# davidbau/rewriting

Measured on NVIDIA H100. Metric: StyleGAN2-256 images/sec, higher is better.
Workload: dtype bf16x3 (3-term split bf16 operands, fp32 accumulate; fp32 in/out)

## Files before the change

rewriting_b200/csrc/conv_tc.cu:

```cuda
#include <cstdlib>
#include <cstring>

#include "rw_common.cuh"
#include "rw_kernels.h"

namespace rw {

namespace {

constexpr int BM = 128;
constexpr int BN = 128;
constexpr int BK = 32;
constexpr int MMA_K = 16;
constexpr int kStages = 7;
constexpr int kNumThreads = 384;
constexpr int kTmaWarp = 8;
constexpr uint32_t kProducerRegs = 40;
constexpr uint32_t kConsumerRegs = 232;
constexpr int kCluster = 2;
constexpr int kChunkKB = 16;

struct ConvSmem {
  static constexpr int kABytes = BM * BK * 2;
  static constexpr int kBBytes = BN * BK * 2;
  static constexpr int kStageBytes = 2 * kABytes + 2 * kBBytes;
  static constexpr int kTotal = kStages * kStageBytes + 512  + 256 ;
};
static_assert(ConvSmem::kTotal <= 232448, "conv_tc: shared memory over the per-block limit");

struct Barriers {
  uint64_t full[kStages];
  uint64_t empty[kStages];
};

__device__ __forceinline__ void decode_tile(int tile, int nphase, int nsched, int& ph, int& mn) {
  mn = tile / nphase;
  ph = tile - mn * nphase;
  if (nphase > 1) ph = (ph + ((nsched % nphase) == 0 ? tile / nsched : mn)) % nphase;
}

template <int EPI, bool PROF>
__global__ void __launch_bounds__(kNumThreads, 1)
conv_tc_kernel(const __grid_constant__ CUtensorMap map_a_hi,
               const __grid_constant__ CUtensorMap map_a_lo,
               const __grid_constant__ CUtensorMap map_w_hi,
               const __grid_constant__ CUtensorMap map_w_lo, const ConvTcParams p) {
  extern __shared__ uint8_t smem_raw[];
  uint8_t* smem = reinterpret_cast<uint8_t*>((reinterpret_cast<uintptr_t>(smem_raw) + 511) &
                                             ~static_cast<uintptr_t>(511));
  using S = ConvSmem;
  Barriers* bars = reinterpret_cast<Barriers*>(smem + kStages * S::kStageBytes);

  const int warp = __shfl_sync(0xffffffffu, static_cast<int>(threadIdx.x >> 5), 0);
  const int lane = threadIdx.x & 31;
  const int rank = static_cast<int>(cluster_ctarank());
  const int nsched = static_cast<int>(num_clusters_x());
  const int first_unit = static_cast<int>(cluster_id_x());

  const int m_tiles = (p.rows + BM - 1) / BM;
  const int n_tiles = p.Cout / BN;
  const int mn_units = (m_tiles + kCluster - 1) / kCluster * n_tiles;
  const int num_units = mn_units * p.nphase;
  const int kb_per_tap = p.Cin / BK;

  if (warp == kTmaWarp && lane == 0) {
    tma_prefetch_desc(&map_a_hi);
    tma_prefetch_desc(&map_a_lo);
    tma_prefetch_desc(&map_w_hi);
    tma_prefetch_desc(&map_w_lo);
    for (int s = 0; s < kStages; ++s) {
      mbar_init(&bars->full[s], 1);
      mbar_init(&bars->empty[s], 2 * kCluster);
    }
    fence_mbar_init();
  }
  cluster_sync();

  if (warp < kTmaWarp) {
    setmaxnreg_inc<kConsumerRegs>();
    const int wg = threadIdx.x >> 7;
    const int c = lane & 3;
    const int img = p.Hp * p.Wp;
    auto release = [&](int s) {
      if ((threadIdx.x & 127) == 0) {
#pragma unroll
        for (int r = 0; r < kCluster; ++r) mbar_arrive_cluster(mapa_shared(&bars->empty[s], r));
      }
    };
    auto clk = [] { return static_cast<uint32_t>(clock()); };
    uint32_t prof[6] = {0, 0, 0, 0, 0, 0};
    uint32_t tp0 = 0, tp1 = 0;
    if constexpr (PROF) prof[5] = 0u - clk();
    int stage = 0;
    uint32_t phase = 0;
    for (int unit = first_unit; unit < num_units; unit += nsched) {
      int ph, mn;
      decode_tile(unit, p.nphase, nsched, ph, mn);
      const int num_kb = p.ph_ntaps[ph] * kb_per_tap;
      const int n_tile = mn % n_tiles;
      const int n0 = n_tile * BN;
      const int m0 = ((mn / n_tiles) * kCluster + rank) * BM;

      float acc[64], d[64];
#pragma unroll
      for (int j = 0; j < 64; ++j) acc[j] = 0.f;
      for (int kb0 = 0; kb0 < num_kb; kb0 += kChunkKB) {
        const int kb_end = (kb0 + kChunkKB < num_kb) ? kb0 + kChunkKB : num_kb;
        int held = -1;
        for (int kb = kb0; kb < kb_end; ++kb) {
          if constexpr (PROF) tp0 = clk();
          mbar_wait(&bars->full[stage], phase);
          if constexpr (PROF) { tp1 = clk(); prof[0] += tp1 - tp0; }
          const uint32_t sa = smem_u32(smem + stage * S::kStageBytes);
          const uint64_t da_hi = make_smem_desc(sa + wg * (S::kABytes / 2), 16, 512, 2);
          const uint64_t da_lo = make_smem_desc(sa + S::kABytes + wg * (S::kABytes / 2), 16, 512, 2);
          const uint64_t db_hi = make_smem_desc(sa + 2 * S::kABytes, 16, 512, 2);
          const uint64_t db_lo = make_smem_desc(sa + 2 * S::kABytes + S::kBBytes, 16, 512, 2);
          wgmma_fence();
#pragma unroll
          for (int kk = 0; kk < BK / MMA_K; ++kk) {
            const uint64_t adv = static_cast<uint64_t>((kk * MMA_K * 2) >> 4);
            wgmma_m64n128<0, 0>(d, da_lo + adv, db_hi + adv, ((kb - kb0) | kk) != 0);
            wgmma_m64n128<0, 0>(d, da_hi + adv, db_lo + adv, 1u);
            wgmma_m64n128<0, 0>(d, da_hi + adv, db_hi + adv, 1u);
          }
          wgmma_commit();
          wgmma_wait<1>();
          if (held >= 0) release(held);
          held = stage;
          if (++stage == kStages) { stage = 0; phase ^= 1u; }
          if constexpr (PROF) prof[1] += clk() - tp1;
        }
        if constexpr (PROF) tp0 = clk();
        wgmma_wait<0>();
        release(held);
#pragma unroll
        for (int j = 0; j < 64; ++j) acc[j] += d[j];
        if constexpr (PROF) prof[2] += clk() - tp0;
      }
      if constexpr (PROF) tp0 = clk();

      uint32_t tid;
      asm volatile("mov.u32 %0, %%tid.x;\n" : "=r"(tid));
      const int row0 = m0 + ((tid >> 7) << 6) + (((tid >> 5) & 3) << 4) + ((tid & 31) >> 2);
#pragma unroll
      for (int i = 0; i < 2; ++i) {
        const int prow = row0 + 8 * i;
        const int b = prow / img;
        const int rem = prow - b * img;
        const int yy = rem / p.Wp;
        const int xx = rem - yy * p.Wp;
        const int Hv = p.ph_Hv[ph], Wv = p.ph_Wv[ph];
        const bool in_rows = prow < p.rows;
        const bool valid = in_rows && (yy < Hv) && (xx < Wv);
        const float* scl = (p.scale_bo && in_rows) ? p.scale_bo + static_cast<size_t>(b) * p.Cout : nullptr;
        float* outp = (p.out != nullptr && p.out_mode == 0 && valid)
                          ? p.out + p.ph_out_ofs[ph] + static_cast<size_t>(b) * p.out_sb +
                                static_cast<size_t>(yy) * p.out_sy + static_cast<size_t>(xx) * p.out_sx
                          : nullptr;
        if (EPI == 1 || !valid) {
          if (scl && (EPI == 1 || p.out_mode == 1)) {
#pragma unroll
            for (int j = 0; j < 16; ++j) {
              const float2 sv = __ldg(reinterpret_cast<const float2*>(scl + n0 + 8 * j + 2 * c));
              acc[4 * j + 2 * i] *= sv.x;
              acc[4 * j + 2 * i + 1] *= sv.y;
            }
          }
          if (EPI == 1 && outp) {
#pragma unroll
            for (int j = 0; j < 16; ++j)
#pragma unroll
              for (int e = 0; e < 2; ++e)
                outp[static_cast<size_t>(n0 + 8 * j + 2 * c + e) * p.out_sc] = acc[4 * j + 2 * i + e];
          }
        } else {
          float nz = 0.f;
          if (p.noise != nullptr)
            nz = __ldg(p.noise_w) * __ldg(p.noise + static_cast<size_t>(b) * p.noise_bstride +
                                          static_cast<size_t>(yy) * Wv + xx);
          const float act_gain = p.act_gain != 0.f ? p.act_gain : 1.4142135623730951f;
          if (scl) {
            const float* sc = scl + n0 + 2 * c;
#pragma unroll
            for (int j = 0; j < 16; ++j)
#pragma unroll
              for (int e = 0; e < 2; ++e) acc[4 * j + 2 * i + e] *= __ldg(sc + 8 * j + e);
          }
#pragma unroll
          for (int j = 0; j < 16; ++j)
#pragma unroll
            for (int e = 0; e < 2; ++e) acc[4 * j + 2 * i + e] += nz;
          if (p.bias) {
            const float* bi = p.bias + n0 + 2 * c;
#pragma unroll
            for (int j = 0; j < 16; ++j)
#pragma unroll
              for (int e = 0; e < 2; ++e) acc[4 * j + 2 * i + e] += __ldg(bi + 8 * j + e);
          }
          if (p.act) {
#pragma unroll
            for (int j = 0; j < 32; ++j) {
              float& t = acc[4 * (j >> 1) + 2 * i + (j & 1)];
              t = (t > 0.f ? t : 0.2f * t) * act_gain;
            }
          }
          if (outp) {
#pragma unroll
            for (int j = 0; j < 16; ++j)
#pragma unroll
              for (int e = 0; e < 2; ++e)
                outp[static_cast<size_t>(n0 + 8 * j + 2 * c + e) * p.out_sc] = acc[4 * j + 2 * i + e];
          }
        }
        if (EPI == 0 && p.rgb_w != nullptr) {
          const float* rw0 = p.rgb_w + (static_cast<size_t>(valid ? b : 0) * 3) * p.Cout + n0 + 2 * c;
          const float* rw1 = rw0 + p.Cout;
          const float* rw2 = rw1 + p.Cout;
#pragma unroll
          for (int half = 0; half < 2; ++half) {
            float r0 = 0.f, r1 = 0.f, r2 = 0.f;
            if (valid) {
#pragma unroll
              for (int j = 8 * half; j < 8 * half + 8; ++j)
#pragma unroll
                for (int e = 0; e < 2; ++e) {
                  const float t = acc[4 * j + 2 * i + e];
                  r0 = fmaf(__ldg(rw0 + 8 * j + e), t, r0);
                  r1 = fmaf(__ldg(rw1 + 8 * j + e), t, r1);
                  r2 = fmaf(__ldg(rw2 + 8 * j + e), t, r2);
                }
            }
#pragma unroll
            for (int s = 1; s < 4; s <<= 1) {
              r0 += __shfl_xor_sync(0xffffffffu, r0, s);
              r1 += __shfl_xor_sync(0xffffffffu, r1, s);
              r2 += __shfl_xor_sync(0xffffffffu, r2, s);
            }
            if (valid && c == 0) {
              const size_t hw = static_cast<size_t>(Hv) * Wv;
              float* rp = p.rgb_part + ((static_cast<size_t>(n_tile * 2 + half) * p.B + b) * 3) * hw +
                          static_cast<size_t>(yy) * Wv + xx;
              rp[0] = r0;
              rp[hw] = r1;
              rp[2 * hw] = r2;
            }
          }
        }
        if (p.out != nullptr && p.out_mode == 1 && in_rows) {
          float* orow = p.out + (static_cast<size_t>(ph) * p.rows + prow) * p.Cout + n0 + 2 * c;
#pragma unroll
          for (int j = 0; j < 16; ++j)
            *reinterpret_cast<float2*>(orow + 8 * j) = make_float2(acc[4 * j + 2 * i], acc[4 * j + 2 * i + 1]);
        }
        if (EPI == 0 && p.next_hi != nullptr && in_rows) {
          const float* ns = p.next_scale + static_cast<size_t>(valid ? b : 0) * p.Cout + n0 + 2 * c;
          const size_t ofs = static_cast<size_t>(prow) * p.Cout + n0 + 2 * c;
          uint32_t* nh = reinterpret_cast<uint32_t*>(static_cast<__nv_bfloat16*>(p.next_hi) + ofs);
          uint32_t* nl = reinterpret_cast<uint32_t*>(static_cast<__nv_bfloat16*>(p.next_lo) + ofs);
#pragma unroll
          for (int j = 0; j < 16; ++j) {
            float k0 = 0.f, k1 = 0.f;
            if (valid) {
              const float2 sv = __ldg(reinterpret_cast<const float2*>(ns + 8 * j));
              k0 = sv.x * acc[4 * j + 2 * i];
              k1 = sv.y * acc[4 * j + 2 * i + 1];
            }
            const __nv_bfloat162 hh = __floats2bfloat162_rn(k0, k1);
            const float2 hf = __bfloat1622float2(hh);
            const __nv_bfloat162 ll = __floats2bfloat162_rn(k0 - hf.x, k1 - hf.y);
            nh[4 * j] = *reinterpret_cast<const uint32_t*>(&hh);
            nl[4 * j] = *reinterpret_cast<const uint32_t*>(&ll);
          }
        }
      }
      if constexpr (PROF) { prof[3] += clk() - tp0; prof[4] += 1; }
    }
    if constexpr (PROF) {
      prof[5] += clk();
      if (lane == 0) {
        long long* dst = p.debug_prof + (static_cast<size_t>(blockIdx.x) * 8 + warp) * 8;
#pragma unroll
        for (int i = 0; i < 8; ++i) dst[i] = i < 6 ? prof[i] : 0;
      }
    }
  } else {
    setmaxnreg_dec<kProducerRegs>();
    if (warp == kTmaWarp && lane == 0) {
      constexpr uint16_t kMask = (1u << kCluster) - 1;
      constexpr int kBSlice = BN / kCluster;
      const uint32_t b_off = 2 * S::kABytes + rank * (S::kBBytes / kCluster);
      int stage = 0;
      uint32_t phase = 0;
      for (int unit = first_unit; unit < num_units; unit += nsched) {
        int ph, mn;
        decode_tile(unit, p.nphase, nsched, ph, mn);
        const int n0 = (mn % n_tiles) * BN + rank * kBSlice;
        const int m0 = ((mn / n_tiles) * kCluster + rank) * BM;
        for (int t = 0; t < p.ph_ntaps[ph]; ++t) {
          const int arow = m0 + p.ph_shift[ph][t];
          const int wcol = p.ph_kofs[ph][t];
          const int acol = p.ph_acol[ph][t];
          for (int kb = 0; kb < kb_per_tap; ++kb) {
            mbar_wait(&bars->empty[stage], phase ^ 1u);
            uint8_t* st = smem + stage * S::kStageBytes;
            mbar_expect_tx(&bars->full[stage], S::kStageBytes);
            tma_load_2d(st, &map_a_hi, &bars->full[stage], acol + kb * BK, arow);
            tma_load_2d(st + S::kABytes, &map_a_lo, &bars->full[stage], acol + kb * BK, arow);
            tma_load_2d_multicast(st + b_off, &map_w_hi, &bars->full[stage], wcol + kb * BK, n0,
                                  kMask);
            tma_load_2d_multicast(st + b_off + S::kBBytes, &map_w_lo, &bars->full[stage],
                                  wcol + kb * BK, n0, kMask);
            if (++stage == kStages) { stage = 0; phase ^= 1u; }
          }
        }
      }
    }
    __syncwarp();
  }
  cluster_sync();
}

}

template <int EPI, bool PROF>
static int conv_tc_launch_epi(const ConvTcParams& p, const void* a_hi, const void* a_lo,
                              const void* w_hi, const void* w_lo, int wk_total,
                              cudaStream_t stream) {
  CUtensorMap ma_hi, ma_lo, mw_hi, mw_lo;
  int rc;
  const uint64_t a_cols = p.a_cols > 0 ? p.a_cols : p.Cin;
  const uint64_t a_dims[2] = {a_cols, static_cast<uint64_t>(p.rows)}, a_str[1] = {a_cols * 2};
  const uint64_t w_dims[2] = {static_cast<uint64_t>(wk_total), static_cast<uint64_t>(p.Cout)};
  const uint64_t w_str[1] = {static_cast<uint64_t>(wk_total) * 2};
  const uint32_t a_box[2] = {BK, BM}, w_box[2] = {BK, BN / kCluster};
  if ((rc = make_tmap_nd_bf16(&ma_hi, a_hi, 2, a_dims, a_str, a_box, nullptr, 3))) return rc;
  if ((rc = make_tmap_nd_bf16(&ma_lo, a_lo, 2, a_dims, a_str, a_box, nullptr, 3))) return rc;
  if ((rc = make_tmap_nd_bf16(&mw_hi, w_hi, 2, w_dims, w_str, w_box, nullptr, 3))) return rc;
  if ((rc = make_tmap_nd_bf16(&mw_lo, w_lo, 2, w_dims, w_str, w_box, nullptr, 3))) return rc;

  cudaLaunchConfig_t cfg = {};
  cudaLaunchAttribute attr[1];
  attr[0].id = cudaLaunchAttributeClusterDimension;
  attr[0].val.clusterDim.x = kCluster;
  attr[0].val.clusterDim.y = 1;
  attr[0].val.clusterDim.z = 1;
  cfg.blockDim = dim3(kNumThreads);
  cfg.dynamicSmemBytes = ConvSmem::kTotal;
  cfg.stream = stream;
  cfg.attrs = attr;
  cfg.numAttrs = 1;
  static int max_clusters = 0;
  if (max_clusters == 0) {
    rc = check_cuda(cudaFuncSetAttribute(conv_tc_kernel<EPI, PROF>,
                                         cudaFuncAttributeMaxDynamicSharedMemorySize, ConvSmem::kTotal),
                    "conv_tc smem attr");
    if (rc) return rc;
    cfg.gridDim = dim3(kCluster * (device_sm_count() / kCluster));
    rc = check_cuda(cudaOccupancyMaxActiveClusters(&max_clusters, conv_tc_kernel<EPI, PROF>, &cfg),
                    "conv_tc cluster occupancy");
    if (rc) return rc;
    if (max_clusters < 1) {
      set_last_error("conv_tc: no cluster of %d CTAs fits on the device", kCluster);
      return RW_ERR_UNSUPPORTED;
    }
  }
  const int m_tiles = (p.rows + BM - 1) / BM;
  const int n_tiles = p.Cout / BN;
  const int num_units = (m_tiles + kCluster - 1) / kCluster * n_tiles * p.nphase;
  const int clusters = max_clusters < num_units ? max_clusters : num_units;
  cfg.gridDim = dim3(kCluster * clusters);
  rc = check_cuda(cudaLaunchKernelEx(&cfg, conv_tc_kernel<EPI, PROF>, ma_hi, ma_lo, mw_hi, mw_lo, p),
                  "conv_tc launch");
  if (rc) return rc;
  return check_cuda(cudaGetLastError(), "conv_tc launch");
}

int conv_tc_launch(const ConvTcParams& p, const void* a_hi, const void* a_lo, const void* w_hi,
                   const void* w_lo, int wk_total, cudaStream_t stream) {
  if (p.Cin % 64 != 0 || p.Cout % BN != 0 || p.nphase < 1 || p.nphase > 4 || p.rows <= 0) {
    set_last_error("conv_tc: unsupported shape Cin=%d Cout=%d nphase=%d rows=%d", p.Cin, p.Cout,
                   p.nphase, p.rows);
    return RW_ERR_BAD_ARG;
  }
  for (int i = 0; i < p.nphase; ++i)
    if (p.ph_ntaps[i] < 1 || p.ph_ntaps[i] > 9) {
      set_last_error("conv_tc: phase %d has %d taps", i, p.ph_ntaps[i]);
      return RW_ERR_BAD_ARG;
    }
  const bool lean = !p.noise && !p.bias && !p.act && !p.rgb_w && !p.rgb_part && !p.next_hi &&
                    p.out != nullptr && (reinterpret_cast<uintptr_t>(p.scale_bo) & 7u) == 0;
  if (p.debug_prof) return conv_tc_launch_epi<0, true>(p, a_hi, a_lo, w_hi, w_lo, wk_total, stream);
  if (lean) return conv_tc_launch_epi<1, false>(p, a_hi, a_lo, w_hi, w_lo, wk_total, stream);
  return conv_tc_launch_epi<0, false>(p, a_hi, a_lo, w_hi, w_lo, wk_total, stream);
}

}
```

Measured before the change: 1570.

## Offload conv epilogue to dedicated warpgroup via shared-memory staging buffers

```diff
diff --git a/rewriting_b200/csrc/conv_tc.cu b/rewriting_b200/csrc/conv_tc.cu
--- a/rewriting_b200/csrc/conv_tc.cu
+++ b/rewriting_b200/csrc/conv_tc.cu
@@ -12,11 +12,13 @@
 constexpr int BN = 128;
 constexpr int BK = 32;
 constexpr int MMA_K = 16;
-constexpr int kStages = 7;
-constexpr int kNumThreads = 384;
+constexpr int kStages = 5;
+constexpr int kNumThreads = 512;
 constexpr int kTmaWarp = 8;
-constexpr uint32_t kProducerRegs = 40;
-constexpr uint32_t kConsumerRegs = 232;
+constexpr int kEpiWarp0 = 12;
+constexpr uint32_t kConsumerRegs = 184;
+constexpr uint32_t kProducerRegs = 24;
+constexpr uint32_t kEpilogueRegs = 120;
 constexpr int kCluster = 2;
 constexpr int kChunkKB = 16;
 
@@ -24,14 +26,34 @@
   static constexpr int kABytes = BM * BK * 2;
   static constexpr int kBBytes = BN * BK * 2;
   static constexpr int kStageBytes = 2 * kABytes + 2 * kBBytes;
-  static constexpr int kTotal = kStages * kStageBytes + 512  + 256 ;
+  static constexpr int kHalfBytes = (BM / 2) * BN * 4;
+  static constexpr int kStagingOfs = kStages * kStageBytes;
+  static constexpr int kBarOfs = kStagingOfs + 2 * kHalfBytes;
+  static constexpr int kTotal = kBarOfs + 512  + 256 ;
 };
 static_assert(ConvSmem::kTotal <= 232448, "conv_tc: shared memory over the per-block limit");
 
 struct Barriers {
   uint64_t full[kStages];
   uint64_t empty[kStages];
+  uint64_t staged[2];
+  uint64_t drained[2];
 };
+static_assert(sizeof(Barriers) <= 256, "conv_tc: barriers over their shared-memory slot");
+
+__device__ __forceinline__ int staged_ofs(int r, int q, int c, int j) {
+  return r * BN + (((2 * j) ^ q) << 2) + 2 * (c & 1);
+}
+
+__device__ __forceinline__ void store_strided(float* o, long long sc, const float (&v)[32]) {
+  const long long sc8 = 8 * sc;
+#pragma unroll
+  for (int j = 0; j < 16; ++j) {
+    o[0] = v[2 * j];
+    o[sc] = v[2 * j + 1];
+    o += sc8;
+  }
+}
 
 __device__ __forceinline__ void decode_tile(int tile, int nphase, int nsched, int& ph, int& mn) {
   mn = tile / nphase;
@@ -49,7 +71,8 @@
   uint8_t* smem = reinterpret_cast<uint8_t*>((reinterpret_cast<uintptr_t>(smem_raw) + 511) &
                                              ~static_cast<uintptr_t>(511));
   using S = ConvSmem;
-  Barriers* bars = reinterpret_cast<Barriers*>(smem + kStages * S::kStageBytes);
+  float* staging = reinterpret_cast<float*>(smem + S::kStagingOfs);
+  Barriers* bars = reinterpret_cast<Barriers*>(smem + S::kBarOfs);
 
   const int warp = __shfl_sync(0xffffffffu, static_cast<int>(threadIdx.x >> 5), 0);
   const int lane = threadIdx.x & 31;
@@ -72,34 +95,37 @@
       mbar_init(&bars->full[s], 1);
       mbar_init(&bars->empty[s], 2 * kCluster);
     }
+    for (int h = 0; h < 2; ++h) {
+      mbar_init(&bars->staged[h], 128);
+      mbar_init(&bars->drained[h], 128);
+    }
     fence_mbar_init();
   }
   cluster_sync();
 
+  const int frow = ((warp & 3) << 4) + (lane >> 2);
+  const int c = lane & 3;
+  const int q = (lane >> 2) ^ (c >> 1);
+  auto clk = [] { return static_cast<uint32_t>(clock()); };
   if (warp < kTmaWarp) {
     setmaxnreg_inc<kConsumerRegs>();
     const int wg = threadIdx.x >> 7;
-    const int c = lane & 3;
-    const int img = p.Hp * p.Wp;
+    float* stg = staging + wg * (S::kHalfBytes / 4);
     auto release = [&](int s) {
       if ((threadIdx.x & 127) == 0) {
 #pragma unroll
         for (int r = 0; r < kCluster; ++r) mbar_arrive_cluster(mapa_shared(&bars->empty[s], r));
       }
     };
-    auto clk = [] { return static_cast<uint32_t>(clock()); };
-    uint32_t prof[6] = {0, 0, 0, 0, 0, 0};
+    uint32_t prof[8] = {0, 0, 0, 0, 0, 0, 0, 0};
     uint32_t tp0 = 0, tp1 = 0;
-    if constexpr (PROF) prof[5] = 0u - clk();
+    if constexpr (PROF) prof[6] = 0u - clk();
     int stage = 0;
-    uint32_t phase = 0;
+    uint32_t phase = 0, hphase = 0;
     for (int unit = first_unit; unit < num_units; unit += nsched) {
       int ph, mn;
       decode_tile(unit, p.nphase, nsched, ph, mn);
       const int num_kb = p.ph_ntaps[ph] * kb_per_tap;
-      const int n_tile = mn % n_tiles;
-      const int n0 = n_tile * BN;
-      const int m0 = ((mn / n_tiles) * kCluster + rank) * BM;
 
       float acc[64], d[64];
 #pragma unroll
@@ -139,149 +165,183 @@
         if constexpr (PROF) prof[2] += clk() - tp0;
       }
       if constexpr (PROF) tp0 = clk();
-
-      uint32_t tid;
-      asm volatile("mov.u32 %0, %%tid.x;\n" : "=r"(tid));
-      const int row0 = m0 + ((tid >> 7) << 6) + (((tid >> 5) & 3) << 4) + ((tid & 31) >> 2);
-#pragma unroll
-      for (int i = 0; i < 2; ++i) {
-        const int prow = row0 + 8 * i;
-        const int b = prow / img;
-        const int rem = prow - b * img;
-        const int yy = rem / p.Wp;
-        const int xx = rem - yy * p.Wp;
-        const int Hv = p.ph_Hv[ph], Wv = p.ph_Wv[ph];
-        const bool in_rows = prow < p.rows;
-        const bool valid = in_rows && (yy < Hv) && (xx < Wv);
-        const float* scl = (p.scale_bo && in_rows) ? p.scale_bo + static_cast<size_t>(b) * p.Cout : nullptr;
-        float* outp = (p.out != nullptr && p.out_mode == 0 && valid)
-                          ? p.out + p.ph_out_ofs[ph] + static_cast<size_t>(b) * p.out_sb +
-                                static_cast<size_t>(yy) * p.out_sy + static_cast<size_t>(xx) * p.out_sx
-                          : nullptr;
-        if (EPI == 1 || !valid) {
-          if (scl && (EPI == 1 || p.out_mode == 1)) {
+      mbar_wait(&bars->drained[wg], hphase ^ 1u);
+      if constexpr (PROF) { tp1 = clk(); prof[3] += tp1 - tp0; }
+#pragma unroll
+      for (int i = 0; i < 2; ++i)
+#pragma unroll
+        for (int j = 0; j < 16; ++j)
+          *reinterpret_cast<float2*>(stg + staged_ofs(frow + 8 * i, q, c, j)) =
+              make_float2(acc[4 * j + 2 * i], acc[4 * j + 2 * i + 1]);
+      mbar_arrive(&bars->staged[wg]);
+      hphase ^= 1u;
+      if constexpr (PROF) { prof[4] += clk() - tp1; prof[5] += 1; }
+    }
+    if constexpr (PROF) {
+      prof[6] += clk();
+      if (lane == 0) {
+        long long* dst = p.debug_prof + (static_cast<size_t>(blockIdx.x) * 16 + warp) * 8;
+#pragma unroll
+        for (int i = 0; i < 8; ++i) dst[i] = prof[i];
+      }
+    }
+  } else if (warp >= kEpiWarp0) {
+    setmaxnreg_dec<kEpilogueRegs>();
+    const int img = p.Hp * p.Wp;
+    uint32_t prof[8] = {0, 0, 0, 0, 0, 0, 0, 0};
+    uint32_t tp0 = 0, tp1 = 0;
+    if constexpr (PROF) prof[6] = 0u - clk();
+    uint32_t hphase = 0;
+    for (int unit = first_unit; unit < num_units; unit += nsched) {
+      int ph, mn;
+      decode_tile(unit, p.nphase, nsched, ph, mn);
+      const int n_tile = mn % n_tiles;
+      const int n0 = n_tile * BN;
+      const int m0 = ((mn / n_tiles) * kCluster + rank) * BM;
+#pragma unroll 1
+      for (int h = 0; h < 2; ++h) {
+        const float* stg = staging + h * (S::kHalfBytes / 4);
+        if constexpr (PROF) tp0 = clk();
+        mbar_wait(&bars->staged[h], hphase);
+        if constexpr (PROF) { tp1 = clk(); prof[0] += tp1 - tp0; }
+#pragma unroll
+        for (int i = 0; i < 2; ++i) {
+          float acc[32];
+#pragma unroll
+          for (int j = 0; j < 16; ++j) {
+            const float2 v = *reinterpret_cast<const float2*>(stg + staged_ofs(frow + 8 * i, q, c, j));
+            acc[2 * j] = v.x;
+            acc[2 * j + 1] = v.y;
+          }
+          if (i == 1) mbar_arrive(&bars->drained[h]);
+          const int prow = m0 + 64 * h + frow + 8 * i;
+          const int b = prow / img;
+          const int rem = prow - b * img;
+          const int yy = rem / p.Wp;
+          const int xx = rem - yy * p.Wp;
+          const int Hv = p.ph_Hv[ph], Wv = p.ph_Wv[ph];
+          const bool in_rows = prow < p.rows;
+          const bool valid = in_rows && (yy < Hv) && (xx < Wv);
+          const float* scl = (p.scale_bo && in_rows) ? p.scale_bo + static_cast<size_t>(b) * p.Cout : nullptr;
+          float* outp = (p.out != nullptr && p.out_mode == 0 && valid)
+                            ? p.out + p.ph_out_ofs[ph] + static_cast<size_t>(b) * p.out_sb +
+                                  static_cast<size_t>(yy) * p.out_sy + static_cast<size_t>(xx) * p.out_sx
+                            : nullptr;
+          if (EPI == 1 || !valid) {
+            if (scl && (EPI == 1 || p.out_mode == 1)) {
+#pragma unroll
+              for (int j = 0; j < 16; ++j) {
+                const float2 sv = __ldg(reinterpret_cast<const float2*>(scl + n0 + 8 * j + 2 * c));
+                acc[2 * j] *= sv.x;
+                acc[2 * j + 1] *= sv.y;
+              }
+            }
+            if (EPI == 1 && outp) store_strided(outp + static_cast<size_t>(n0 + 2 * c) * p.out_sc, p.out_sc, acc);
+          } else {
+            float nz = 0.f;
+            if (p.noise != nullptr)
+              nz = __ldg(p.noise_w) * __ldg(p.noise + static_cast<size_t>(b) * p.noise_bstride +
+                                            static_cast<size_t>(yy) * Wv + xx);
+            const float act_gain = p.act_gain != 0.f ? p.act_gain : 1.4142135623730951f;
+            if (scl) {
+              const float* sc = scl + n0 + 2 * c;
+#pragma unroll
+              for (int j = 0; j < 16; ++j)
+#pragma unroll
+                for (int e = 0; e < 2; ++e) acc[2 * j + e] *= __ldg(sc + 8 * j + e);
+            }
+#pragma unroll
+            for (int j = 0; j < 16; ++j)
+#pragma unroll
+              for (int e = 0; e < 2; ++e) acc[2 * j + e] += nz;
+            if (p.bias) {
+              const float* bi = p.bias + n0 + 2 * c;
+#pragma unroll
+              for (int j = 0; j < 16; ++j)
+#pragma unroll
+                for (int e = 0; e < 2; ++e) acc[2 * j + e] += __ldg(bi + 8 * j + e);
+            }
+            if (p.act) {
+#pragma unroll
+              for (int j = 0; j < 32; ++j) {
+                float& t = acc[j];
+                t = (t > 0.f ? t : 0.2f * t) * act_gain;
+              }
+            }
+            if (outp) store_strided(outp + static_cast<size_t>(n0 + 2 * c) * p.out_sc, p.out_sc, acc);
+          }
+          if (EPI == 0 && p.rgb_w != nullptr) {
+            const float* rw0 = p.rgb_w + (static_cast<size_t>(valid ? b : 0) * 3) * p.Cout + n0 + 2 * c;
+            const float* rw1 = rw0 + p.Cout;
+            const float* rw2 = rw1 + p.Cout;
+#pragma unroll
+            for (int half = 0; half < 2; ++half) {
+              float r0 = 0.f, r1 = 0.f, r2 = 0.f;
+              if (valid) {
+#pragma unroll
+                for (int j = 8 * half; j < 8 * half + 8; ++j)
+#pragma unroll
+                  for (int e = 0; e < 2; ++e) {
+                    const float t = acc[2 * j + e];
+                    r0 = fmaf(__ldg(rw0 + 8 * j + e), t, r0);
+                    r1 = fmaf(__ldg(rw1 + 8 * j + e), t, r1);
+                    r2 = fmaf(__ldg(rw2 + 8 * j + e), t, r2);
+                  }
+              }
+#pragma unroll
+              for (int s = 1; s < 4; s <<= 1) {
+                r0 += __shfl_xor_sync(0xffffffffu, r0, s);
+                r1 += __shfl_xor_sync(0xffffffffu, r1, s);
+                r2 += __shfl_xor_sync(0xffffffffu, r2, s);
+              }
+              if (valid && c == 0) {
+                const size_t hw = static_cast<size_t>(Hv) * Wv;
+                float* rp = p.rgb_part + ((static_cast<size_t>(n_tile * 2 + half) * p.B + b) * 3) * hw +
+                            static_cast<size_t>(yy) * Wv + xx;
+                rp[0] = r0;
+                rp[hw] = r1;
+                rp[2 * hw] = r2;
+              }
+            }
+          }
+          if (p.out != nullptr && p.out_mode == 1 && in_rows) {
+            float* orow = p.out + (static_cast<size_t>(ph) * p.rows + prow) * p.Cout + n0 + 2 * c;
+#pragma unroll
+            for (int j = 0; j < 16; ++j)
+              *reinterpret_cast<float2*>(orow + 8 * j) = make_float2(acc[2 * j], acc[2 * j + 1]);
+          }
+          if (EPI == 0 && p.next_hi != nullptr && in_rows) {
+            const float* ns = p.next_scale + static_cast<size_t>(valid ? b : 0) * p.Cout + n0 + 2 * c;
+            const size_t ofs = static_cast<size_t>(prow) * p.Cout + n0 + 2 * c;
+            uint32_t* nh = reinterpret_cast<uint32_t*>(static_cast<__nv_bfloat16*>(p.next_hi) + ofs);
+            uint32_t* nl = reinterpret_cast<uint32_t*>(static_cast<__nv_bfloat16*>(p.next_lo) + ofs);
 #pragma unroll
             for (int j = 0; j < 16; ++j) {
-              const float2 sv = __ldg(reinterpret_cast<const float2*>(scl + n0 + 8 * j + 2 * c));
-              acc[4 * j + 2 * i] *= sv.x;
-              acc[4 * j + 2 * i + 1] *= sv.y;
-            }
-          }
-          if (EPI == 1 && outp) {
-#pragma unroll
-            for (int j = 0; j < 16; ++j)
-#pragma unroll
-              for (int e = 0; e < 2; ++e)
-                outp[static_cast<size_t>(n0 + 8 * j + 2 * c + e) * p.out_sc] = acc[4 * j + 2 * i + e];
-          }
-        } else {
-          float nz = 0.f;
-          if (p.noise != nullptr)
-            nz = __ldg(p.noise_w) * __ldg(p.noise + static_cast<size_t>(b) * p.noise_bstride +
-                                          static_cast<size_t>(yy) * Wv + xx);
-          const float act_gain = p.act_gain != 0.f ? p.act_gain : 1.4142135623730951f;
-          if (scl) {
-            const float* sc = scl + n0 + 2 * c;
-#pragma unroll
-            for (int j = 0; j < 16; ++j)
-#pragma unroll
-              for (int e = 0; e < 2; ++e) acc[4 * j + 2 * i + e] *= __ldg(sc + 8 * j + e);
-          }
-#pragma unroll
-          for (int j = 0; j < 16; ++j)
-#pragma unroll
-            for (int e = 0; e < 2; ++e) acc[4 * j + 2 * i + e] += nz;
-          if (p.bias) {
-            const float* bi = p.bias + n0 + 2 * c;
-#pragma unroll
-            for (int j = 0; j < 16; ++j)
-#pragma unroll
-              for (int e = 0; e < 2; ++e) acc[4 * j + 2 * i + e] += __ldg(bi + 8 * j + e);
-          }
-          if (p.act) {
-#pragma unroll
-            for (int j = 0; j < 32; ++j) {
-              float& t = acc[4 * (j >> 1) + 2 * i + (j & 1)];
-              t = (t > 0.f ? t : 0.2f * t) * act_gain;
-            }
-          }
-          if (outp) {
-#pragma unroll
-            for (int j = 0; j < 16; ++j)
-#pragma unroll
-              for (int e = 0; e < 2; ++e)
-                outp[static_cast<size_t>(n0 + 8 * j + 2 * c + e) * p.out_sc] = acc[4 * j + 2 * i + e];
+              float k0 = 0.f, k1 = 0.f;
+              if (valid) {
+                const float2 sv = __ldg(reinterpret_cast<const float2*>(ns + 8 * j));
+                k0 = sv.x * acc[2 * j];
+                k1 = sv.y * acc[2 * j + 1];
+              }
+              const __nv_bfloat162 hh = __floats2bfloat162_rn(k0, k1);
+              const float2 hf = __bfloat1622float2(hh);
+              const __nv_bfloat162 ll = __floats2bfloat162_rn(k0 - hf.x, k1 - hf.y);
+              nh[4 * j] = *reinterpret_cast<const uint32_t*>(&hh);
+              nl[4 * j] = *reinterpret_cast<const uint32_t*>(&ll);
+            }
           }
         }
-        if (EPI == 0 && p.rgb_w != nullptr) {
-          const float* rw0 = p.rgb_w + (static_cast<size_t>(valid ? b : 0) * 3) * p.Cout + n0 + 2 * c;
-          const float* rw1 = rw0 + p.Cout;
-          const float* rw2 = rw1 + p.Cout;
-#pragma unroll
-          for (int half = 0; half < 2; ++half) {
-            float r0 = 0.f, r1 = 0.f, r2 = 0.f;
-            if (valid) {
-#pragma unroll
-              for (int j = 8 * half; j < 8 * half + 8; ++j)
-#pragma unroll
-                for (int e = 0; e < 2; ++e) {
-                  const float t = acc[4 * j + 2 * i + e];
-                  r0 = fmaf(__ldg(rw0 + 8 * j + e), t, r0);
-                  r1 = fmaf(__ldg(rw1 + 8 * j + e), t, r1);
-                  r2 = fmaf(__ldg(rw2 + 8 * j + e), t, r2);
-                }
-            }
-#pragma unroll
-            for (int s = 1; s < 4; s <<= 1) {
-              r0 += __shfl_xor_sync(0xffffffffu, r0, s);
-              r1 += __shfl_xor_sync(0xffffffffu, r1, s);
-              r2 += __shfl_xor_sync(0xffffffffu, r2, s);
-            }
-            if (valid && c == 0) {
-              const size_t hw = static_cast<size_t>(Hv) * Wv;
-              float* rp = p.rgb_part + ((static_cast<size_t>(n_tile * 2 + half) * p.B + b) * 3) * hw +
-                          static_cast<size_t>(yy) * Wv + xx;
-              rp[0] = r0;
-              rp[hw] = r1;
-              rp[2 * hw] = r2;
-            }
-          }
-        }
-        if (p.out != nullptr && p.out_mode == 1 && in_rows) {
-          float* orow = p.out + (static_cast<size_t>(ph) * p.rows + prow) * p.Cout + n0 + 2 * c;
-#pragma unroll
-          for (int j = 0; j < 16; ++j)
-            *reinterpret_cast<float2*>(orow + 8 * j) = make_float2(acc[4 * j + 2 * i], acc[4 * j + 2 * i + 1]);
-        }
-        if (EPI == 0 && p.next_hi != nullptr && in_rows) {
-          const float* ns = p.next_scale + static_cast<size_t>(valid ? b : 0) * p.Cout + n0 + 2 * c;
-          const size_t ofs = static_cast<size_t>(prow) * p.Cout + n0 + 2 * c;
-          uint32_t* nh = reinterpret_cast<uint32_t*>(static_cast<__nv_bfloat16*>(p.next_hi) + ofs);
-          uint32_t* nl = reinterpret_cast<uint32_t*>(static_cast<__nv_bfloat16*>(p.next_lo) + ofs);
-#pragma unroll
-          for (int j = 0; j < 16; ++j) {
-            float k0 = 0.f, k1 = 0.f;
-            if (valid) {
-              const float2 sv = __ldg(reinterpret_cast<const float2*>(ns + 8 * j));
-              k0 = sv.x * acc[4 * j + 2 * i];
-              k1 = sv.y * acc[4 * j + 2 * i + 1];
-            }
-            const __nv_bfloat162 hh = __floats2bfloat162_rn(k0, k1);
-            const float2 hf = __bfloat1622float2(hh);
-            const __nv_bfloat162 ll = __floats2bfloat162_rn(k0 - hf.x, k1 - hf.y);
-            nh[4 * j] = *reinterpret_cast<const uint32_t*>(&hh);
-            nl[4 * j] = *reinterpret_cast<const uint32_t*>(&ll);
-          }
-        }
-      }
-      if constexpr (PROF) { prof[3] += clk() - tp0; prof[4] += 1; }
+        if constexpr (PROF) prof[1] += clk() - tp1;
+      }
+      hphase ^= 1u;
+      if constexpr (PROF) prof[5] += 1;
     }
     if constexpr (PROF) {
-      prof[5] += clk();
+      prof[6] += clk();
       if (lane == 0) {
-        long long* dst = p.debug_prof + (static_cast<size_t>(blockIdx.x) * 8 + warp) * 8;
-#pragma unroll
-        for (int i = 0; i < 8; ++i) dst[i] = i < 6 ? prof[i] : 0;
+        long long* dst = p.debug_prof + (static_cast<size_t>(blockIdx.x) * 16 + warp) * 8;
+#pragma unroll
+        for (int i = 0; i < 8; ++i) dst[i] = prof[i];
       }
     }
   } else {
@@ -317,6 +377,13 @@
       }
     }
     __syncwarp();
+    if constexpr (PROF) {
+      if (lane == 0) {
+        long long* dst = p.debug_prof + (static_cast<size_t>(blockIdx.x) * 16 + warp) * 8;
+#pragma unroll
+        for (int i = 0; i < 8; ++i) dst[i] = 0;
+      }
+    }
   }
   cluster_sync();
 }
```

Result: no change. 1585 (median of 6 runs) (+1.0%).

## Offload conv epilogue to dedicated warpgroup via shared-memory accumulator staging

Applied to the files above, without the earlier changes.

```diff
diff --git a/rewriting_b200/csrc/conv_tc.cu b/rewriting_b200/csrc/conv_tc.cu
--- a/rewriting_b200/csrc/conv_tc.cu
+++ b/rewriting_b200/csrc/conv_tc.cu
@@ -12,11 +12,17 @@
 constexpr int BN = 128;
 constexpr int BK = 32;
 constexpr int MMA_K = 16;
-constexpr int kStages = 7;
-constexpr int kNumThreads = 384;
-constexpr int kTmaWarp = 8;
+constexpr int kStages = 5;
+constexpr int kNumThreads = 512;
+constexpr int kEpiWarp = 8;
+constexpr int kTmaWarp = 12;
+constexpr uint32_t kConsumerRegs = 176;
+constexpr uint32_t kEpilogueRegs = 120;
 constexpr uint32_t kProducerRegs = 40;
-constexpr uint32_t kConsumerRegs = 232;
+static_assert(kConsumerRegs % 8 == 0 && kEpilogueRegs % 8 == 0 && kProducerRegs % 8 == 0 &&
+                  2 * kConsumerRegs + kEpilogueRegs + kProducerRegs <=
+                      (kNumThreads / 128) * (65536 / kNumThreads),
+              "conv_tc: setmaxnreg split over the launch allocation");
 constexpr int kCluster = 2;
 constexpr int kChunkKB = 16;
 
@@ -24,19 +30,32 @@
   static constexpr int kABytes = BM * BK * 2;
   static constexpr int kBBytes = BN * BK * 2;
   static constexpr int kStageBytes = 2 * kABytes + 2 * kBBytes;
-  static constexpr int kTotal = kStages * kStageBytes + 512  + 256 ;
+  static constexpr int kStagingBytes = BM * BN * 4;
+  static constexpr int kStagingOfs = kStages * kStageBytes;
+  static constexpr int kTotal =
+      kStagingOfs + kStagingBytes + 512  + 256 ;
 };
 static_assert(ConvSmem::kTotal <= 232448, "conv_tc: shared memory over the per-block limit");
 
 struct Barriers {
   uint64_t full[kStages];
   uint64_t empty[kStages];
+  uint64_t acc_full;
+  uint64_t acc_empty;
 };
+static_assert(sizeof(Barriers) <= 256, "conv_tc: barriers over their shared-memory slot");
 
 __device__ __forceinline__ void decode_tile(int tile, int nphase, int nsched, int& ph, int& mn) {
   mn = tile / nphase;
   ph = tile - mn * nphase;
   if (nphase > 1) ph = (ph + ((nsched % nphase) == 0 ? tile / nsched : mn)) % nphase;
+}
+
+__device__ __forceinline__ void store_prof(long long* debug_prof, int warp,
+                                           const uint32_t (&prof)[7]) {
+  long long* dst = debug_prof + (static_cast<size_t>(blockIdx.x) * (kNumThreads / 32) + warp) * 8;
+#pragma unroll
+  for (int i = 0; i < 8; ++i) dst[i] = i < 7 ? prof[i] : 0;
 }
 
 template <int EPI, bool PROF>
@@ -49,7 +68,8 @@
   uint8_t* smem = reinterpret_cast<uint8_t*>((reinterpret_cast<uintptr_t>(smem_raw) + 511) &
                                              ~static_cast<uintptr_t>(511));
   using S = ConvSmem;
-  Barriers* bars = reinterpret_cast<Barriers*>(smem + kStages * S::kStageBytes);
+  float2* staging = reinterpret_cast<float2*>(smem + S::kStagingOfs);
+  Barriers* bars = reinterpret_cast<Barriers*>(smem + S::kStagingOfs + S::kStagingBytes);
 
   const int warp = __shfl_sync(0xffffffffu, static_cast<int>(threadIdx.x >> 5), 0);
   const int lane = threadIdx.x & 31;
@@ -72,15 +92,15 @@
       mbar_init(&bars->full[s], 1);
       mbar_init(&bars->empty[s], 2 * kCluster);
     }
+    mbar_init(&bars->acc_full, 256);
+    mbar_init(&bars->acc_empty, 128);
     fence_mbar_init();
   }
   cluster_sync();
 
-  if (warp < kTmaWarp) {
+  if (warp < kEpiWarp) {
     setmaxnreg_inc<kConsumerRegs>();
     const int wg = threadIdx.x >> 7;
-    const int c = lane & 3;
-    const int img = p.Hp * p.Wp;
     auto release = [&](int s) {
       if ((threadIdx.x & 127) == 0) {
 #pragma unroll
@@ -88,18 +108,15 @@
       }
     };
     auto clk = [] { return static_cast<uint32_t>(clock()); };
-    uint32_t prof[6] = {0, 0, 0, 0, 0, 0};
+    uint32_t prof[7] = {0, 0, 0, 0, 0, 0, 0};
     uint32_t tp0 = 0, tp1 = 0;
-    if constexpr (PROF) prof[5] = 0u - clk();
+    if constexpr (PROF) prof[6] = 0u - clk();
     int stage = 0;
-    uint32_t phase = 0;
+    uint32_t phase = 0, acc_phase = 0;
     for (int unit = first_unit; unit < num_units; unit += nsched) {
       int ph, mn;
       decode_tile(unit, p.nphase, nsched, ph, mn);
       const int num_kb = p.ph_ntaps[ph] * kb_per_tap;
-      const int n_tile = mn % n_tiles;
-      const int n0 = n_tile * BN;
-      const int m0 = ((mn / n_tiles) * kCluster + rank) * BM;
 
       float acc[64], d[64];
 #pragma unroll
@@ -139,150 +156,196 @@
         if constexpr (PROF) prof[2] += clk() - tp0;
       }
       if constexpr (PROF) tp0 = clk();
-
-      uint32_t tid;
-      asm volatile("mov.u32 %0, %%tid.x;\n" : "=r"(tid));
-      const int row0 = m0 + ((tid >> 7) << 6) + (((tid >> 5) & 3) << 4) + ((tid & 31) >> 2);
-#pragma unroll
-      for (int i = 0; i < 2; ++i) {
-        const int prow = row0 + 8 * i;
-        const int b = prow / img;
-        const int rem = prow - b * img;
-        const int yy = rem / p.Wp;
-        const int xx = rem - yy * p.Wp;
-        const int Hv = p.ph_Hv[ph], Wv = p.ph_Wv[ph];
-        const bool in_rows = prow < p.rows;
-        const bool valid = in_rows && (yy < Hv) && (xx < Wv);
-        const float* scl = (p.scale_bo && in_rows) ? p.scale_bo + static_cast<size_t>(b) * p.Cout : nullptr;
-        float* outp = (p.out != nullptr && p.out_mode == 0 && valid)
-                          ? p.out + p.ph_out_ofs[ph] + static_cast<size_t>(b) * p.out_sb +
-                                static_cast<size_t>(yy) * p.out_sy + static_cast<size_t>(xx) * p.out_sx
-                          : nullptr;
-        if (EPI == 1 || !valid) {
-          if (scl && (EPI == 1 || p.out_mode == 1)) {
+      mbar_wait(&bars->acc_empty, acc_phase ^ 1u);
+      if constexpr (PROF) { tp1 = clk(); prof[3] += tp1 - tp0; }
+      float2* stg = staging + threadIdx.x;
+#pragma unroll
+      for (int j = 0; j < 16; ++j)
+#pragma unroll
+        for (int i = 0; i < 2; ++i)
+          stg[(j * 2 + i) * 256] = make_float2(acc[4 * j + 2 * i], acc[4 * j + 2 * i + 1]);
+      mbar_arrive(&bars->acc_full);
+      acc_phase ^= 1u;
+      if constexpr (PROF) { prof[4] += clk() - tp1; prof[5] += 1; }
+    }
+    if constexpr (PROF) {
+      prof[6] += clk();
+      if (lane == 0) store_prof(p.debug_prof, warp, prof);
+    }
+  } else if (warp < kTmaWarp) {
+    setmaxnreg_dec<kEpilogueRegs>();
+    const int img = p.Hp * p.Wp;
+    auto clk = [] { return static_cast<uint32_t>(clock()); };
+    uint32_t prof[7] = {0, 0, 0, 0, 0, 0, 0};
+    uint32_t tp0 = 0, tp1 = 0;
+    if constexpr (PROF) prof[6] = 0u - clk();
+    uint32_t acc_phase = 0;
+    for (int unit = first_unit; unit < num_units; unit += nsched) {
+      int ph, mn;
+      decode_tile(unit, p.nphase, nsched, ph, mn);
+      const int n_tile = mn % n_tiles;
+      const int n0 = n_tile * BN;
+      const int m0 = ((mn / n_tiles) * kCluster + rank) * BM;
+      if constexpr (PROF) tp0 = clk();
+      mbar_wait(&bars->acc_full, acc_phase);
+      if constexpr (PROF) { tp1 = clk(); prof[0] += tp1 - tp0; }
+#pragma unroll 1
+      for (int h = 0; h < 2; ++h) {
+        float acc[64];
+#pragma unroll
+        for (int i = 0; i < 2; ++i) {
+          uint32_t tid;
+          asm volatile("mov.u32 %0, %%tid.x;\n" : "=r"(tid));
+          const int ct = static_cast<int>(tid & 127) + 128 * h;
+          const int c = ct & 3;
+          const float2* stg = staging + ct;
+#pragma unroll
+          for (int j = 0; j < 16; ++j) {
+            const float2 v = stg[(j * 2 + i) * 256];
+            acc[4 * j + 2 * i] = v.x;
+            acc[4 * j + 2 * i + 1] = v.y;
+          }
+          if (h == 1 && i == 1) mbar_arrive(&bars->acc_empty);
+          const int prow =
+              m0 + ((ct >> 7) << 6) + (((ct >> 5) & 3) << 4) + ((ct & 31) >> 2) + 8 * i;
+          const int b = prow / img;
+          const int rem = prow - b * img;
+          const int yy = rem / p.Wp;
+          const int xx = rem - yy * p.Wp;
+          const int Hv = p.ph_Hv[ph], Wv = p.ph_Wv[ph];
+          const bool in_rows = prow < p.rows;
+          const bool valid = in_rows && (yy < Hv) && (xx < Wv);
+          const float* scl =
+              (p.scale_bo && in_rows) ? p.scale_bo + static_cast<size_t>(b) * p.Cout : nullptr;
+          float* outp = (p.out != nullptr && p.out_mode == 0 && valid)
+                            ? p.out + p.ph_out_ofs[ph] + static_cast<size_t>(b) * p.out_sb +
+                                  static_cast<size_t>(yy) * p.out_sy +
+                                  static_cast<size_t>(xx) * p.out_sx
+                            : nullptr;
+          if (EPI == 1 || !valid) {
+            if (scl && (EPI == 1 || p.out_mode == 1)) {
+#pragma unroll
+              for (int j = 0; j < 16; ++j) {
+                const float2 sv = __ldg(reinterpret_cast<const float2*>(scl + n0 + 8 * j + 2 * c));
+                acc[4 * j + 2 * i] *= sv.x;
+                acc[4 * j + 2 * i + 1] *= sv.y;
+              }
+            }
+            if (EPI == 1 && outp) {
+#pragma unroll
+              for (int j = 0; j < 16; ++j)
+#pragma unroll
+                for (int e = 0; e < 2; ++e)
+                  outp[static_cast<size_t>(n0 + 8 * j + 2 * c + e) * p.out_sc] = acc[4 * j + 2 * i + e];
+            }
+          } else {
+            float nz = 0.f;
+            if (p.noise != nullptr)
+              nz = __ldg(p.noise_w) * __ldg(p.noise + static_cast<size_t>(b) * p.noise_bstride +
+                                            static_cast<size_t>(yy) * Wv + xx);
+            const float act_gain = p.act_gain != 0.f ? p.act_gain : 1.4142135623730951f;
+            if (scl) {
+              const float* sc = scl + n0 + 2 * c;
+#pragma unroll
+              for (int j = 0; j < 16; ++j)
+#pragma unroll
+                for (int e = 0; e < 2; ++e) acc[4 * j + 2 * i + e] *= __ldg(sc + 8 * j + e);
+            }
+#pragma unroll
+            for (int j = 0; j < 16; ++j)
+#pragma unroll
+              for (int e = 0; e < 2; ++e) acc[4 * j + 2 * i + e] += nz;
+            if (p.bias) {
+              const float* bi = p.bias + n0 + 2 * c;
+#pragma unroll
+              for (int j = 0; j < 16; ++j)
+#pragma unroll
+                for (int e = 0; e < 2; ++e) acc[4 * j + 2 * i + e] += __ldg(bi + 8 * j + e);
+            }
+            if (p.act) {
+#pragma unroll
+              for (int j = 0; j < 32; ++j) {
+                float& t = acc[4 * (j >> 1) + 2 * i + (j & 1)];
+                t = (t > 0.f ? t : 0.2f * t) * act_gain;
+              }
+            }
+            if (outp) {
+#pragma unroll
+              for (int j = 0; j < 16; ++j)
+#pragma unroll
+                for (int e = 0; e < 2; ++e)
+                  outp[static_cast<size_t>(n0 + 8 * j + 2 * c + e) * p.out_sc] = acc[4 * j + 2 * i + e];
+            }
+          }
+          if (EPI == 0 && p.rgb_w != nullptr) {
+            const float* rw0 = p.rgb_w + (static_cast<size_t>(valid ? b : 0) * 3) * p.Cout + n0 + 2 * c;
+            const float* rw1 = rw0 + p.Cout;
+            const float* rw2 = rw1 + p.Cout;
+#pragma unroll
+            for (int half = 0; half < 2; ++half) {
+              float r0 = 0.f, r1 = 0.f, r2 = 0.f;
+              if (valid) {
+#pragma unroll
+                for (int j = 8 * half; j < 8 * half + 8; ++j)
+#pragma unroll
+                  for (int e = 0; e < 2; ++e) {
+                    const float t = acc[4 * j + 2 * i + e];
+                    r0 = fmaf(__ldg(rw0 + 8 * j + e), t, r0);
+                    r1 = fmaf(__ldg(rw1 + 8 * j + e), t, r1);
+                    r2 = fmaf(__ldg(rw2 + 8 * j + e), t, r2);
+                  }
+              }
+#pragma unroll
+              for (int s = 1; s < 4; s <<= 1) {
+                r0 += __shfl_xor_sync(0xffffffffu, r0, s);
+                r1 += __shfl_xor_sync(0xffffffffu, r1, s);
+                r2 += __shfl_xor_sync(0xffffffffu, r2, s);
+              }
+              if (valid && c == 0) {
+                const size_t hw = static_cast<size_t>(Hv) * Wv;
+                float* rp = p.rgb_part + ((static_cast<size_t>(n_tile * 2 + half) * p.B + b) * 3) * hw +
+                            static_cast<size_t>(yy) * Wv + xx;
+                rp[0] = r0;
+                rp[hw] = r1;
+                rp[2 * hw] = r2;
+              }
+            }
+          }
+          if (p.out != nullptr && p.out_mode == 1 && in_rows) {
+            float* orow = p.out + (static_cast<size_t>(ph) * p.rows + prow) * p.Cout + n0 + 2 * c;
+#pragma unroll
+            for (int j = 0; j < 16; ++j)
+              *reinterpret_cast<float2*>(orow + 8 * j) =
+                  make_float2(acc[4 * j + 2 * i], acc[4 * j + 2 * i + 1]);
+          }
+          if (EPI == 0 && p.next_hi != nullptr && in_rows) {
+            const float* ns = p.next_scale + static_cast<size_t>(valid ? b : 0) * p.Cout + n0 + 2 * c;
+            const size_t ofs = static_cast<size_t>(prow) * p.Cout + n0 + 2 * c;
+            uint32_t* nh = reinterpret_cast<uint32_t*>(static_cast<__nv_bfloat16*>(p.next_hi) + ofs);
+            uint32_t* nl = reinterpret_cast<uint32_t*>(static_cast<__nv_bfloat16*>(p.next_lo) + ofs);
 #pragma unroll
             for (int j = 0; j < 16; ++j) {
-              const float2 sv = __ldg(reinterpret_cast<const float2*>(scl + n0 + 8 * j + 2 * c));
-              acc[4 * j + 2 * i] *= sv.x;
-              acc[4 * j + 2 * i + 1] *= sv.y;
-            }
-          }
-          if (EPI == 1 && outp) {
-#pragma unroll
-            for (int j = 0; j < 16; ++j)
-#pragma unroll
-              for (int e = 0; e < 2; ++e)
-                outp[static_cast<size_t>(n0 + 8 * j + 2 * c + e) * p.out_sc] = acc[4 * j + 2 * i + e];
-          }
-        } else {
-          float nz = 0.f;
-          if (p.noise != nullptr)
-            nz = __ldg(p.noise_w) * __ldg(p.noise + static_cast<size_t>(b) * p.noise_bstride +
-                                          static_cast<size_t>(yy) * Wv + xx);
-          const float act_gain = p.act_gain != 0.f ? p.act_gain : 1.4142135623730951f;
-          if (scl) {
-            const float* sc = scl + n0 + 2 * c;
-#pragma unroll
-            for (int j = 0; j < 16; ++j)
-#pragma unroll
-              for (int e = 0; e < 2; ++e) acc[4 * j + 2 * i + e] *= __ldg(sc + 8 * j + e);
-          }
-#pragma unroll
-          for (int j = 0; j < 16; ++j)
-#pragma unroll
-            for (int e = 0; e < 2; ++e) acc[4 * j + 2 * i + e] += nz;
-          if (p.bias) {
-            const float* bi = p.bias + n0 + 2 * c;
-#pragma unroll
-            for (int j = 0; j < 16; ++j)
-#pragma unroll
-              for (int e = 0; e < 2; ++e) acc[4 * j + 2 * i + e] += __ldg(bi + 8 * j + e);
-          }
-          if (p.act) {
-#pragma unroll
-            for (int j = 0; j < 32; ++j) {
-              float& t = acc[4 * (j >> 1) + 2 * i + (j & 1)];
-              t = (t > 0.f ? t : 0.2f * t) * act_gain;
-            }
-          }
-          if (outp) {
-#pragma unroll
-            for (int j = 0; j < 16; ++j)
-#pragma unroll
-              for (int e = 0; e < 2; ++e)
-                outp[static_cast<size_t>(n0 + 8 * j + 2 * c + e) * p.out_sc] = acc[4 * j + 2 * i + e];
-          }
-        }
-        if (EPI == 0 && p.rgb_w != nullptr) {
-          const float* rw0 = p.rgb_w + (static_cast<size_t>(valid ? b : 0) * 3) * p.Cout + n0 + 2 * c;
-          const float* rw1 = rw0 + p.Cout;
-          const float* rw2 = rw1 + p.Cout;
-#pragma unroll
-          for (int half = 0; half < 2; ++half) {
-            float r0 = 0.f, r1 = 0.f, r2 = 0.f;
-            if (valid) {
-#pragma unroll
-              for (int j = 8 * half; j < 8 * half + 8; ++j)
-#pragma unroll
-                for (int e = 0; e < 2; ++e) {
-                  const float t = acc[4 * j + 2 * i + e];
-                  r0 = fmaf(__ldg(rw0 + 8 * j + e), t, r0);
-                  r1 = fmaf(__ldg(rw1 + 8 * j + e), t, r1);
-                  r2 = fmaf(__ldg(rw2 + 8 * j + e), t, r2);
-                }
-            }
-#pragma unroll
-            for (int s = 1; s < 4; s <<= 1) {
-              r0 += __shfl_xor_sync(0xffffffffu, r0, s);
-              r1 += __shfl_xor_sync(0xffffffffu, r1, s);
-              r2 += __shfl_xor_sync(0xffffffffu, r2, s);
-            }
-            if (valid && c == 0) {
-              const size_t hw = static_cast<size_t>(Hv) * Wv;
-              float* rp = p.rgb_part + ((static_cast<size_t>(n_tile * 2 + half) * p.B + b) * 3) * hw +
-                          static_cast<size_t>(yy) * Wv + xx;
-              rp[0] = r0;
-              rp[hw] = r1;
-              rp[2 * hw] = r2;
-            }
-          }
-        }
-        if (p.out != nullptr && p.out_mode == 1 && in_rows) {
-          float* orow = p.out + (static_cast<size_t>(ph) * p.rows + prow) * p.Cout + n0 + 2 * c;
-#pragma unroll
-          for (int j = 0; j < 16; ++j)
-            *reinterpret_cast<float2*>(orow + 8 * j) = make_float2(acc[4 * j + 2 * i], acc[4 * j + 2 * i + 1]);
-        }
-        if (EPI == 0 && p.next_hi != nullptr && in_rows) {
-          const float* ns = p.next_scale + static_cast<size_t>(valid ? b : 0) * p.Cout + n0 + 2 * c;
-          const size_t ofs = static_cast<size_t>(prow) * p.Cout + n0 + 2 * c;
-          uint32_t* nh = reinterpret_cast<uint32_t*>(static_cast<__nv_bfloat16*>(p.next_hi) + ofs);
-          uint32_t* nl = reinterpret_cast<uint32_t*>(static_cast<__nv_bfloat16*>(p.next_lo) + ofs);
-#pragma unroll
-          for (int j = 0; j < 16; ++j) {
-            float k0 = 0.f, k1 = 0.f;
-            if (valid) {
-              const float2 sv = __ldg(reinterpret_cast<const float2*>(ns + 8 * j));
-              k0 = sv.x * acc[4 * j + 2 * i];
-              k1 = sv.y * acc[4 * j + 2 * i + 1];
-            }
-            const __nv_bfloat162 hh = __floats2bfloat162_rn(k0, k1);
-            const float2 hf = __bfloat1622float2(hh);
-            const __nv_bfloat162 ll = __floats2bfloat162_rn(k0 - hf.x, k1 - hf.y);
-            nh[4 * j] = *reinterpret_cast<const uint32_t*>(&hh);
-            nl[4 * j] = *reinterpret_cast<const uint32_t*>(&ll);
+              float k0 = 0.f, k1 = 0.f;
+              if (valid) {
+                const float2 sv = __ldg(reinterpret_cast<const float2*>(ns + 8 * j));
+                k0 = sv.x * acc[4 * j + 2 * i];
+                k1 = sv.y * acc[4 * j + 2 * i + 1];
+              }
+              const __nv_bfloat162 hh = __floats2bfloat162_rn(k0, k1);
+              const float2 hf = __bfloat1622float2(hh);
+              const __nv_bfloat162 ll = __floats2bfloat162_rn(k0 - hf.x, k1 - hf.y);
+              nh[4 * j] = *reinterpret_cast<const uint32_t*>(&hh);
+              nl[4 * j] = *reinterpret_cast<const uint32_t*>(&ll);
+            }
           }
         }
       }
-      if constexpr (PROF) { prof[3] += clk() - tp0; prof[4] += 1; }
+      acc_phase ^= 1u;
+      if constexpr (PROF) { prof[1] += clk() - tp1; prof[5] += 1; }
     }
     if constexpr (PROF) {
-      prof[5] += clk();
-      if (lane == 0) {
-        long long* dst = p.debug_prof + (static_cast<size_t>(blockIdx.x) * 8 + warp) * 8;
-#pragma unroll
-        for (int i = 0; i < 8; ++i) dst[i] = i < 6 ? prof[i] : 0;
-      }
+      prof[6] += clk();
+      if (lane == 0) store_prof(p.debug_prof, warp, prof);
     }
   } else {
     setmaxnreg_dec<kProducerRegs>();
```

After: 1569 before, 1600 after, median of 6. 2.0% higher.
